# dazchi/gym-uav-collision-avoidance

Hardware: AMD Instinct MI355X
Metric: env-steps/s (higher is better)
Workload: dtype f32+f64

## Files before the change

### gym_uav_collision_avoidance_amd/csrc/uavx_device.hpp

```cpp
#pragma once
#include <hip/hip_runtime.h>
#include <stdint.h>

namespace uavx {

constexpr int kWave = 64;
#ifndef UAVX_BLOCK
#define UAVX_BLOCK 64
#endif
constexpr int kBlock = UAVX_BLOCK;
constexpr int kWavesPerBlock = kBlock / kWave;
constexpr float kPi = 3.14159265358979323846f;
constexpr float kInvPi = 0.318309886183790671538f;
constexpr float kTwoPi = 6.28318530717958647692f;
constexpr float kInvTwoPi = 0.159154943091895335769f;

__device__ __forceinline__ void wave_lds_sync() {
    __builtin_amdgcn_fence(__ATOMIC_RELEASE, "wavefront");
    __builtin_amdgcn_wave_barrier();
    __builtin_amdgcn_fence(__ATOMIC_ACQUIRE, "wavefront");
}

using rsrc_t = __amdgpu_buffer_rsrc_t;
typedef unsigned int u32x4 __attribute__((ext_vector_type(4)));
typedef unsigned int u32x2 __attribute__((ext_vector_type(2)));
constexpr int kAuxSc1 = 16;

__device__ __forceinline__ rsrc_t make_rsrc(const void *base, uint32_t bytes) {
    return __builtin_amdgcn_make_buffer_rsrc(const_cast<void *>(base),  0, (int)bytes, 0x00020000);
}
__device__ __forceinline__ void store16_wt(rsrc_t r, uint32_t byte_off, float4 v) {
    u32x4 d = {__float_as_uint(v.x), __float_as_uint(v.y), __float_as_uint(v.z), __float_as_uint(v.w)};
    __builtin_amdgcn_raw_buffer_store_b128(d, r, (int)byte_off, 0, kAuxSc1);
}
__device__ __forceinline__ void store16_wt(rsrc_t r, uint32_t byte_off, double2 v) {
    const unsigned long long a = __double_as_longlong(v.x), b = __double_as_longlong(v.y);
    u32x4 d = {(unsigned)a, (unsigned)(a >> 32), (unsigned)b, (unsigned)(b >> 32)};
    __builtin_amdgcn_raw_buffer_store_b128(d, r, (int)byte_off, 0, kAuxSc1);
}
__device__ __forceinline__ void store8_wt(rsrc_t r, uint32_t byte_off, float2 v) {
    u32x2 d = {__float_as_uint(v.x), __float_as_uint(v.y)};
    __builtin_amdgcn_raw_buffer_store_b64(d, r, (int)byte_off, 0, kAuxSc1);
}

typedef const __attribute__((address_space(4))) char *karg_ptr;
__device__ __forceinline__ karg_ptr late_kargs() {
    karg_ptr ka = (karg_ptr)__builtin_amdgcn_kernarg_segment_ptr();
    asm volatile("" : "+s"(ka));
    return ka;
}
template <class T>
__device__ __forceinline__ T late_karg(uint32_t byte_off, karg_ptr ka = late_kargs()) {
    return *(const __attribute__((address_space(4))) T *)(ka + byte_off);
}

__device__ __forceinline__ float sqrt_rn(float s) {
    if (__builtin_expect(__any((__float_as_uint(s) - 1u) < 0x0F7FFFFFu), 0)) return sqrtf(s);
    const float r = __builtin_amdgcn_sqrtf(s);
    const float lo = __uint_as_float(__float_as_uint(r) - 1u), hi = __uint_as_float(__float_as_uint(r) + 1u);
    const float e_lo = fmaf(-lo, r, s), e_hi = fmaf(-hi, r, s);
    float out = (e_lo <= 0.f) ? lo : r;
// ... 229 lines not shown
```

### gym_uav_collision_avoidance_amd/csrc/uavx_multi_host.hpp

```cpp

extern "C" {

int uavx_version(void) { return UAVX_VERSION; }

#ifndef UAVX_SRC_HASH
#define UAVX_SRC_HASH ""
#endif
static const char kBuildInfo[] = "UAVX_SRC_HASH=" UAVX_SRC_HASH;
const char *uavx_build_info(void) { return kBuildInfo + 14; }
int uavx_polar_commands(const void *actions, int action_dtype, int64_t n, float scale, double *out, void *stream) {
    if (n < 0 || (n > 0 && (!actions || !out))) return UAVX_ERR_INVALID_ARG;
    if (action_dtype != UAVX_F32 && action_dtype != UAVX_F64) return UAVX_ERR_INVALID_ARG;
    if ((reinterpret_cast<uintptr_t>(actions) & (action_dtype == UAVX_F64 ? 15u : 7u)) || (reinterpret_cast<uintptr_t>(out) & 15u))
        return UAVX_ERR_INVALID_ARG;
    if (n == 0) return UAVX_OK;
    const auto kernel = action_dtype == UAVX_F64 ? &polar_commands_kernel<true> : &polar_commands_kernel<false>;
    return launch_items((uavx_handle *)nullptr, kernel, n, static_cast<hipStream_t>(stream), actions, n, scale, reinterpret_cast<double2 *>(out));
}

const char *uavx_strerror(int status) {
    switch (status) {
        case UAVX_OK: return "ok";
        case UAVX_ERR_INVALID_ARG: return "invalid argument";
        case UAVX_ERR_HIP: return "HIP runtime error";
// ... 29 lines not shown
    h->gw = B > 0 ? 1 : pick_group_waves(N);
    if (const char *gv = getenv("UAVX_GW")) {
        const int w = atoi(gv);
        if (w >= 1 && w <= 4 && B == 0 && !(N == 1 || N == 2 || N == 4 || N == 5 || N == 8)) h->gw = w;
    }
    p.epw = std::min(kWave * h->gw / N, kExtSlots / (N + B));
    p.magic = 65536 / N + 1;
    p.E = num_envs;
    p.env_offset = env_offset;
    h->ext = B > 0;
    {
        const int lps = std::min(kHintJobs, std::max(1, kWave * h->gw / (N + B)));
        h->prefetch_every = std::max(1, 64 * lps / std::max(1, p.epw));
    }
    apply_body_rule(h);
    h->levels.l[0] = make_level(*cfg, nullptr, N, B);

    DeviceGuard guard(device);
    hipError_t e = guard.err;
    if (e != hipSuccess) { delete h; return UAVX_ERR_HIP; }
    const size_t A = (size_t)num_envs * N, E = (size_t)num_envs;
    size_t off = 0;
    const size_t o_pos = off;  off = align_up(off + A * sizeof(float2), 256);
    const size_t o_ovr = off;  off = align_up(off + A * sizeof(float), 256);
    const size_t o_vel = off;  off = align_up(off + A * sizeof(double2), 256);
    const size_t o_goal = off; off = align_up(off + A * sizeof(Goal), 256);
    const size_t o_steps = off; off = align_up(off + E * sizeof(uint4), 256);
    const size_t o_wsteps = off; off = align_up(off + ((E + p.epw - 1) / p.epw) * 4, 256);
    const size_t o_reach = off; off = align_up(off + E * 4, 256);
    const size_t o_coll = off;  off = align_up(off + E * 4, 256);
    const size_t o_nonfin = off; off = align_up(off + E * 4, 256);
    const size_t o_finc = off;  off = align_up(off + E * sizeof(uint4), 256);
    const size_t o_finr = off;  off = align_up(off + E * sizeof(float2), 256);
    const size_t o_bpos = off;  off = align_up(off + E * (size_t)B * sizeof(float2), 256);
    const size_t o_bleg = off;  off = align_up(off + E * (size_t)B * sizeof(float4), 256);
    const size_t o_lcur = off;  off = align_up(off + E, 256);
    const size_t o_lnext = off; off = align_up(off + E, 256);
    const size_t o_levels = off; off = align_up(off + sizeof(LevelTable), 256);
    const size_t o_sagent = off; off = align_up(off + 2 * A * sizeof(float4), 256);
    const size_t o_sbpos = off;  off = align_up(off + 2 * E * (size_t)B * sizeof(float2), 256);
    const size_t o_sbleg = off;  off = align_up(off + 2 * E * (size_t)B * sizeof(float4), 256);
    const size_t o_stag = off;   off = align_up(off + 2 * E * sizeof(uint4), 256);
    const size_t o_hint = off;   off = align_up(off + ((E + p.epw - 1) / p.epw + 1) * kHintJobs * sizeof(uint2), 256);
    static_assert(sizeof(size_t) >= 8, "64-bit host");
    if (o_pos != 0 || o_wsteps >= (size_t(1) << 32)) { delete h; return UAVX_ERR_UNSUPPORTED; }
    h->off_vel = (uint32_t)o_vel; h->off_goal = (uint32_t)o_goal; h->off_rec = (uint32_t)o_steps; h->off_wsteps = (uint32_t)o_wsteps;
    if (p.epw > 255 || p.nslots > 255) { delete h; return UAVX_ERR_UNSUPPORTED; }
    e = hipMalloc(&h->slab, off);
    if (e != hipSuccess) { delete h; return UAVX_ERR_ALLOC; }
    h->slab_bytes = off;
    e = hipMemset(h->slab, 0, off);
    if (e != hipSuccess) { (void)hipFree(h->slab); delete h; return UAVX_ERR_HIP; }
    char *b = static_cast<char *>(h->slab);
    p.pos = reinterpret_cast<float2 *>(b + o_pos);
    p.prev_ovr = reinterpret_cast<float *>(b + o_ovr);
    p.vel = reinterpret_cast<double2 *>(b + o_vel);
    p.goal = reinterpret_cast<Goal *>(b + o_goal);
    p.env_rec = reinterpret_cast<uint4 *>(b + o_steps);
    p.wave_steps = reinterpret_cast<uint32_t *>(b + o_wsteps);
    p.reach = reinterpret_cast<uint32_t *>(b + o_reach);
    p.coll = reinterpret_cast<uint32_t *>(b + o_coll);
    p.nonfin = reinterpret_cast<uint32_t *>(b + o_nonfin);
    p.fin_counts = reinterpret_cast<uint4 *>(b + o_finc);
    p.fin_returns = reinterpret_cast<float2 *>(b + o_finr);
    p.body_pos = reinterpret_cast<float2 *>(b + o_bpos);
    p.body_leg = reinterpret_cast<float4 *>(b + o_bleg);
    p.lvl_cur = reinterpret_cast<uint8_t *>(b + o_lcur);
    p.lvl_next = reinterpret_cast<uint8_t *>(b + o_lnext);
    h->levels_dev = reinterpret_cast<LevelParams *>(b + o_levels);
    p.levels = h->levels_dev;
    p.n_levels = 0; p.level_lo = -1; p.level_hi = -1;
    p.stage_agent = reinterpret_cast<float4 *>(b + o_sagent);
    p.stage_bpos = reinterpret_cast<float2 *>(b + o_sbpos);
    p.stage_bleg = reinterpret_cast<float4 *>(b + o_sbleg);
    p.stage_tag = reinterpret_cast<uint4 *>(b + o_stag);
    h->hints = reinterpret_cast<uint2 *>(b + o_hint);
// ... 129 lines not shown
int uavx_num_agents(const uavx_handle *h) { return h ? h->p.N : -1; }
static int launch_observe(uavx_handle *h, float *obs, hipStream_t st) {
    if (h->wide) return launch_items(h, observe64_kernel, h->p.E, st, h->p, h->w, h->wl, obs);
    return dispatch(h, ObserveLaunch{h, wave_grid(h), st, obs});
}

int uavx_observe(uavx_handle *h, float *obs, void *stream) {
    if (!h) return UAVX_ERR_INVALID_ARG;
    if (!obs || (reinterpret_cast<uintptr_t>(obs) & 15u))
        return fail(h, UAVX_ERR_INVALID_ARG, "uavx_observe: obs is NULL or not 16-byte aligned");
    UAVX_ENTER(h);
    return launch_observe(h, obs, static_cast<hipStream_t>(stream));
}

int uavx_reset(uavx_handle *h, const uint8_t *mask, uint64_t seed, float *obs, void *stream) {
    if (!h) return UAVX_ERR_INVALID_ARG;
    UAVX_ENTER(h);
    if (obs && (reinterpret_cast<uintptr_t>(obs) & 15u))
        return fail(h, UAVX_ERR_INVALID_ARG, "uavx_reset: obs not 16-byte aligned");
    if (h->wide && mask)
        return fail(h, UAVX_ERR_UNSUPPORTED, "uavx_reset: a masked reset would mix float32 and float64 episodes in one handle");
    h->wide = false;
    hipStream_t st = static_cast<hipStream_t>(stream);
    const int rc = dispatch(h, ResetLaunch{h, wave_grid(h), st, mask, seed});
    if (rc != UAVX_OK || !obs) return rc;
    return launch_observe(h, obs, st);
}

static int launch_step64(uavx_handle *h, const void *actions, int action_dtype, int action_mode, int track_returns, int evaluate,
                  float *obs, float *rew, uint8_t *done, hipStream_t st) {
    const bool f64 = action_dtype == UAVX_F64;
    const auto kernel = action_mode == UAVX_ACTION_POLAR_REFERENCE ? (f64 ? &step64_ref_kernel<true> : &step64_ref_kernel<false>)
                                                                   : (f64 ? &step64_kernel<true> : &step64_kernel<false>);
    return launch_items(h, kernel, h->p.E, st, h->p, h->w, h->wl, actions, action_mode, track_returns, evaluate, obs, rew, done);
}

int uavx_step_k(uavx_handle *h, int k, const void *actions, int action_dtype, int evaluate, int tape_out, float *obs,
                float *rew, uint8_t *done, void *stream) {
    if (!h) return UAVX_ERR_INVALID_ARG;
    if (!actions || !obs || !rew || !done) return fail(h, UAVX_ERR_INVALID_ARG, "uavx_step: NULL buffer");
    if (k < 1) return fail(h, UAVX_ERR_INVALID_ARG, "uavx_step_k: k < 1");
    if (action_dtype != UAVX_F32 && action_dtype != UAVX_F64)
        return fail(h, UAVX_ERR_INVALID_ARG, "uavx_step: action_dtype must be UAVX_F32 or UAVX_F64");
    if ((reinterpret_cast<uintptr_t>(obs) & 15u) || (reinterpret_cast<uintptr_t>(actions) & (action_dtype == UAVX_F64 ? 15u : 7u)) ||
        (reinterpret_cast<uintptr_t>(rew) & 3u))
        return fail(h, UAVX_ERR_INVALID_ARG, "uavx_step: obs must be 16-byte aligned, actions 8 (float32) / 16 (float64), rew 4");
    UAVX_ENTER(h);
    if (h->wide) {
        if (k != 1) return fail(h, UAVX_ERR_UNSUPPORTED, "uavx_step_k: k > 1 is not available for float64-position episodes");
        return launch_step64(h, actions, action_dtype, UAVX_ACTION_CARTESIAN, 0, evaluate, obs, rew, done,
                             static_cast<hipStream_t>(stream));
    }
    if (h->ext && k != 1)
        return fail(h, UAVX_ERR_UNSUPPORTED, "uavx_step_k: k > 1 is not available with scripted bodies / a curriculum");
    return dispatch(h, StepLaunch{h, wave_grid(h), static_cast<hipStream_t>(stream), actions, action_dtype, evaluate, k, tape_out, obs, rew, done});
}

int uavx_step(uavx_handle *h, const void *actions, int action_dtype, int evaluate, float *obs, float *rew,
              uint8_t *done, void *stream) {
    return uavx_step_k(h, 1, actions, action_dtype, evaluate, 0, obs, rew, done, stream);
}

int uavx_step_ex(uavx_handle *h, const uavx_step_args *a, void *stream) {
    if (!h || !a) return UAVX_ERR_INVALID_ARG;
    if (!a->actions || !a->obs || !a->rew || !a->done) return fail(h, UAVX_ERR_INVALID_ARG, "uavx_step_ex: NULL buffer");
    if (a->action_dtype != UAVX_F32 && a->action_dtype != UAVX_F64)
        return fail(h, UAVX_ERR_INVALID_ARG, "uavx_step_ex: action_dtype must be UAVX_F32 or UAVX_F64");
    if (a->action_mode != UAVX_ACTION_CARTESIAN && a->action_mode != UAVX_ACTION_POLAR &&
        a->action_mode != UAVX_ACTION_POLAR_REFERENCE)
        return fail(h, UAVX_ERR_INVALID_ARG, "uavx_step_ex: unknown action_mode");
    if (a->reset_policy < UAVX_RESET_NEVER || a->reset_policy > UAVX_RESET_ALL_DONE)
        return fail(h, UAVX_ERR_INVALID_ARG, "uavx_step_ex: unknown reset_policy");
    if (a->flags_mode != UAVX_FLAGS_ARRAYS && a->flags_mode != UAVX_FLAGS_IN_DONE)
        return fail(h, UAVX_ERR_INVALID_ARG, "uavx_step_ex: unknown flags_mode");
    if ((reinterpret_cast<uintptr_t>(a->obs) & 15u) || (reinterpret_cast<uintptr_t>(a->actions) & (a->action_dtype == UAVX_F64 ? 15u : 7u)) ||
        (reinterpret_cast<uintptr_t>(a->rew) & 3u))
        return fail(h, UAVX_ERR_INVALID_ARG, "uavx_step_ex: obs must be 16-byte aligned, actions 8 (float32) / 16 (float64), rew 4");
    UAVX_ENTER(h);
    if (h->wide) {
        if (a->reset_policy != UAVX_RESET_NEVER || a->step_cap != 0)
            return fail(h, UAVX_ERR_UNSUPPORTED, "uavx_step_ex: no auto-reset / step cap for float64-position episodes");
        if (a->reset_mask) UAVX_HIP(h, hipMemsetAsync(a->reset_mask, 0, (size_t)h->p.E, static_cast<hipStream_t>(stream)));
        if (a->ended) UAVX_HIP(h, hipMemsetAsync(a->ended, 0, (size_t)h->p.E, static_cast<hipStream_t>(stream)));
        if (a->truncated) UAVX_HIP(h, hipMemsetAsync(a->truncated, 0, (size_t)h->p.E, static_cast<hipStream_t>(stream)));
        return launch_step64(h, a->actions, a->action_dtype, a->action_mode, a->track_returns, a->evaluate, a->obs, a->rew,
                             a->done, static_cast<hipStream_t>(stream));
    }
    StepExtra x;
    x.action_mode = a->action_mode; x.reset_policy = a->reset_policy; x.track_returns = a->track_returns;
    x.step_cap = a->step_cap; x.seed_lo = (uint32_t)a->seed; x.seed_hi = (uint32_t)(a->seed >> 32);
    x.reset_mask = a->reset_mask;
    x.ended = a->ended; x.truncated = a->truncated;
    x.flags_in_done = (a->flags_mode == UAVX_FLAGS_IN_DONE) ? 1 : 0;
    hipStream_t st = static_cast<hipStream_t>(stream);
    const dim3 grid = wave_grid(h);
    const bool resets = a->reset_policy != UAVX_RESET_NEVER || a->step_cap != 0;
    x.use_stage = (h->prefetch_every > 0 && resets) ? 1 : 0;
    x.pf_blocks = 0; x.pf_groups = grid.x;
    x.stage_first = 0; x.step_first = 0;
    x.hints = h->hints;
    const unsigned step_blocks = grid.x / (unsigned)launch_tiles(h);
// ... 21 lines not shown
}
#endif

int uavx_get_nonfinite(uavx_handle *h, uint32_t *counts, void *stream) {
    if (!h || !counts) return UAVX_ERR_INVALID_ARG;
    UAVX_ENTER(h);
    UAVX_HIP(h, hipMemcpyAsync(counts, h->p.nonfin, (size_t)h->p.E * 4, hipMemcpyDeviceToDevice, static_cast<hipStream_t>(stream)));
    return UAVX_OK;
}

int uavx_get_episode_stats(uavx_handle *h, uint32_t *counts, float *returns, void *stream) {
    if (!h) return UAVX_ERR_INVALID_ARG;
    UAVX_ENTER(h);
    return launch_items(h, episode_stats_kernel, h->p.E, static_cast<hipStream_t>(stream), h->p, counts, returns, 0);
}

int uavx_clear_episode_stats(uavx_handle *h, void *stream) {
    if (!h) return UAVX_ERR_INVALID_ARG;
    UAVX_ENTER(h);
    return launch_items(h, episode_stats_kernel, h->p.E, static_cast<hipStream_t>(stream), h->p, (uint32_t *)nullptr, (float *)nullptr, 1);
}

static int wide_exchange(uavx_handle *h, const uavx_state_view &v, const uavx_state_view_f64 &v64, int set, hipStream_t st) {
    const int rc = launch_items(h, wide_exchange_kernel, agent_slots(h), st, h->p, h->w, v, v64, set);
    if (rc != UAVX_OK || !v.counters) return rc;
    {
        uavx_state_view c;
        std::memset(&c, 0, sizeof c);
        c.counters = v.counters;
        return launch_items(h, set ? set_state_kernel : get_state_kernel, agent_slots(h), st, h->p, c);
    }
}

int uavx_get_state(uavx_handle *h, const uavx_state_view *dst, void *stream) {
    if (!h || !dst) return UAVX_ERR_INVALID_ARG;
    UAVX_ENTER(h);
    if (h->wide) return wide_exchange(h, *dst, uavx_state_view_f64{}, 0, static_cast<hipStream_t>(stream));
    return launch_items(h, get_state_kernel, agent_slots(h), static_cast<hipStream_t>(stream), h->p, *dst);
}

int uavx_set_state(uavx_handle *h, const uavx_state_view *src, void *stream) {
    if (!h || !src) return UAVX_ERR_INVALID_ARG;
    UAVX_ENTER(h);
    if (h->wide) return wide_exchange(h, *src, uavx_state_view_f64{}, 1, static_cast<hipStream_t>(stream));
    return launch_items(h, set_state_kernel, agent_slots(h), static_cast<hipStream_t>(stream), h->p, *src);
}

int uavx_get_position_mode(const uavx_handle *h) { return h ? (h->wide ? UAVX_POS_F64 : UAVX_POS_F32) : UAVX_ERR_INVALID_ARG; }

int uavx_set_position_mode(uavx_handle *h, int mode, void *stream) {
    if (!h) return UAVX_ERR_INVALID_ARG;
    if (mode != UAVX_POS_F32 && mode != UAVX_POS_F64) return fail(h, UAVX_ERR_INVALID_ARG, "uavx_set_position_mode: unknown mode");
    UAVX_ENTER(h);
    if ((mode == UAVX_POS_F64) == h->wide) return UAVX_OK;
    if (mode == UAVX_POS_F64 && h->ext)
        return fail(h, UAVX_ERR_UNSUPPORTED, "uavx_set_position_mode: float64-position episodes are not available with scripted bodies / a curriculum");
    hipStream_t st = static_cast<hipStream_t>(stream);
    if (mode == UAVX_POS_F64) {
        if (!h->wide_slab) {
            const size_t A = (size_t)h->p.E * h->p.N;
            const size_t o_tgt = align_up(A * sizeof(double2), 256), o_init = o_tgt + align_up(A * sizeof(double2), 256);
            const size_t o_prev = o_init + align_up(A * sizeof(double), 256), total = o_prev + align_up(A * sizeof(double), 256);
            if (hipMalloc(&h->wide_slab, total) != hipSuccess) {
                h->wide_slab = nullptr;
                return fail(h, UAVX_ERR_ALLOC, "uavx_set_position_mode: hipMalloc of the float64 arrays failed");
            }
            char *b = static_cast<char *>(h->wide_slab);
            h->w.pos = reinterpret_cast<double2 *>(b);
            h->w.tgt = reinterpret_cast<double2 *>(b + o_tgt);
            h->w.init_d = reinterpret_cast<double *>(b + o_init);
            h->w.prev_d = reinterpret_cast<double *>(b + o_prev);
        }
    }
    const int rc = launch_items(h, mode == UAVX_POS_F64 ? widen_state_kernel : narrow_state_kernel, agent_slots(h), st, h->p, h->w);
    if (rc == UAVX_OK) h->wide = (mode == UAVX_POS_F64);
    return rc;
}

int uavx_set_state_f64(uavx_handle *h, const uavx_state_view_f64 *src, void *stream) {
    if (!h || !src) return UAVX_ERR_INVALID_ARG;
    const int rc = uavx_set_position_mode(h, UAVX_POS_F64, stream);
    if (rc != UAVX_OK) return rc;
    UAVX_ENTER(h);
    uavx_state_view none;
    std::memset(&none, 0, sizeof none);
    return wide_exchange(h, none, *src, 1, static_cast<hipStream_t>(stream));
}

int uavx_get_state_f64(uavx_handle *h, const uavx_state_view_f64 *dst, void *stream) {
    if (!h || !dst) return UAVX_ERR_INVALID_ARG;
    if (!h->wide) return fail(h, UAVX_ERR_UNSUPPORTED, "uavx_get_state_f64: the handle is in float32-position mode");
    UAVX_ENTER(h);
    uavx_state_view none;
    std::memset(&none, 0, sizeof none);
    return wide_exchange(h, none, *dst, 0, static_cast<hipStream_t>(stream));
}
// ... 10 lines not shown
```

### gym_uav_collision_avoidance_amd/csrc/uavx_multi_kernels.hpp

```cpp

#ifndef UAVX_EXB
#define UAVX_EXB 8
#endif
#ifndef UAVX_EX8B
#define UAVX_EX8B 8
#endif
#define UAVX_EX_KERNEL step_ex_kernel
#define UAVX_EX_REF false
#include "uavx_step_ex.hpp"
#undef UAVX_EX_KERNEL
#undef UAVX_EX_REF
#define UAVX_EX_KERNEL step_ex_ref_kernel
#define UAVX_EX_REF true
#include "uavx_step_ex.hpp"
#undef UAVX_EX_KERNEL
#undef UAVX_EX_REF

template <int NT, bool ACT64, int W>
__global__ __launch_bounds__(kWave * W) void step_k_kernel(MultiParams p, const void *__restrict__ actions, int evaluate,
                                                           int K, int tape_out, float *__restrict__ obs_out,
                                                           float *__restrict__ rew_out, uint8_t *__restrict__ done_out) {
    using LDS = LdsT<false, W>;
    __shared__ LDS lds;
    const int N = NT ? NT : p.N;
// ... 10 lines not shown
        float o[10], rew;
        uint32_t dn, re, ce;
        step_agent<NT, false>(p, m, lds, s, ax, ay, evaluate, o, rew, dn, re, ce);
        reach_acc += re;
        coll_acc += ce;
        nonfin_acc += !(fabsf(rew) < INFINITY) ? 1u : 0u;
        if (tape_out || k == K - 1) {
            const size_t off = tape_out ? (size_t)k * A : 0;
            if (m.active) {
                (rew_out + off)[m.a] = rew;
                (done_out + off)[m.a] = (uint8_t)dn;
            }
            store_obs_block<NT>(p, m, lds, o, obs_out + off * UAVX_OBS_DIM);
        } else {
            group_sync<LDS::kW>();
        }
    }
    if (m.active) {
        store_agent(p, m.a, s, flags_in);
        if (reach_acc) atomicAdd(&p.reach[m.e], reach_acc);
        if (coll_acc) atomicAdd(&p.coll[m.e], coll_acc);
        if (nonfin_acc) atomicAdd(&p.nonfin[m.e], nonfin_acc);
        if (m.lane == 0) atomicAdd(&p.wave_steps[m.wave], (uint32_t)K);
    }
}

template <int NT, bool EXT, int W>
__global__ __launch_bounds__(kWave * W) void observe_kernel(MultiParams p, float *__restrict__ obs_out) {
    using LDS = LdsT<EXT, W>;
    __shared__ LDS lds;
    const LaneMap m = lane_map<NT, EXT, W>(p);
    AgentRegs s = {};
    if (m.active) load_agent(p, m.a, s);
    const WorldLims w = world_lims<EXT>(p, s.flags);
    const float tdx = s.tx - s.x, tdy = s.ty - s.y;
    const float dist_t = norm32(tdx, tdy);
    const float theta = atan2_fast((float)s.vy, (float)s.vx);
    const float dth = wrap_pi(atan2_fast(tdy, tdx) - theta);
    if (EXT && p.B > 0) stage_bodies<false>(p, m, lds, s.flags, false, 0u, 0u);
    if (m.active) {
        lds.pos[m.rbase + m.i] = make_float4(s.x, s.y, s.x, s.y);
        lds.theta[m.rbase + m.i] = theta;
    }
    group_sync<LDS::kW>();
    const Neigh nb = scan_neighbours<NT, false>(w.sq_sense, m, lds, s.x, s.y);
    const float speed = __builtin_amdgcn_sqrtf((float)fma(s.vy, s.vy, s.vx * s.vx));
    float o[10];
    assemble_obs(p, w, m, lds, nb, s.x, s.y, speed, theta, dist_t, dth, o);
    if (EXT && (s.flags & kFlagInactive)) {
#pragma unroll
        for (int k = 0; k < UAVX_OBS_DIM; k++) o[k] = 0.f;
    }
    store_obs_block<NT>(p, m, lds, o, obs_out);
}

template <int NT, bool EXT, int W>
__global__ __launch_bounds__(kWave * W) void reset_kernel(MultiParams p, const uint8_t *__restrict__ mask, uint64_t seed) {
    using LDS = LdsT<EXT, W>;
    __shared__ LDS lds;
    const LaneMap m = lane_map<NT, EXT, W>(p);
    const bool go = m.active && (!mask || mask[m.e] != 0);
    if (!group_any<W>(go)) return;
    AgentRegs s = {};
    uint4 rec = make_uint4(0, 0, 0, 0);
    if (go) rec = p.env_rec[m.e];
    const uint32_t episode = rec.y & ~kRecEnded;
    EpisodeFold fold = {};
    uint32_t wc = 0;
    if (go && m.i == 0) {
        fold = fold_load(p, m.e);
        wc = p.wave_steps[m.wave];
    }
    reset_envs_wave<NT, EXT>(p, m, lds, go, episode, (uint32_t)seed, (uint32_t)(seed >> 32), s, p.body_pos, p.body_leg, p.lvl_cur);
    if (go) {
        p.pos[m.a] = make_float2(s.x, s.y);
        p.vel[m.a] = make_double2(0.0, 0.0);
        p.goal[m.a] = Goal{s.tx, s.ty, s.init_d, s.flags};
        if (m.i == 0) {
            fold_store(p, m.e, wc - rec.x, make_float2(__uint_as_float(rec.z), __uint_as_float(rec.w)), fold);
            p.env_rec[m.e] = make_uint4(wc, episode + 1u, 0u, 0u);
        }
    }
}

__global__ __launch_bounds__(64) void upload_levels_kernel(LevelParams *dst, LevelTable t) {
    if (threadIdx.x < UAVX_MAX_LEVELS) dst[threadIdx.x] = t.l[threadIdx.x];
}
__global__ __launch_bounds__(kBlock) void env_levels_kernel(MultiParams p, const uint8_t *set_next, uint8_t *get_cur) {
    const int64_t e = (int64_t)blockIdx.x * kBlock + threadIdx.x;
    if (e >= p.E) return;
    if (set_next) p.lvl_next[e] = set_next[e];
    if (get_cur) get_cur[e] = p.lvl_cur[e];
}
__global__ __launch_bounds__(kBlock) void bodies_kernel(MultiParams p, const float *set, float *get) {
    const int64_t i = (int64_t)blockIdx.x * kBlock + threadIdx.x;
    if (i >= p.E * p.B) return;
    if (set) {
        const float *r = set + i * UAVX_BODY_DIM;
        p.body_pos[i] = make_float2(r[0], r[1]);
        p.body_leg[i] = make_float4(r[2], r[3], r[4], r[5]);
    }
    if (get) {
        const float2 q = p.body_pos[i];
        const float4 leg = p.body_leg[i];
        float *r = get + i * UAVX_BODY_DIM;
// ... 106 lines not shown
```

### gym_uav_collision_avoidance_amd/csrc/uavx_multi_launch.hpp

```cpp

namespace {

template <class L>
int dispatch(const uavx_handle *h, const L &l) {
    if (h->ext) {
        switch (h->gw) {
            case 2: return l.template run<0, true, 2>();
            case 3: return l.template run<0, true, 3>();
            case 4: return l.template run<0, true, 4>();
            default: return l.template run<0, true, 1>();
        }
    }
    switch (h->p.N) {
        case 1: return l.template run<1, false, 1>();
        case 2: return l.template run<2, false, 1>();
        case 4: return l.template run<4, false, 1>();
        case 5: return l.template run<5, false, 1>();
        case 8: return l.template run<8, false, 1>();
        default: break;
    }
    switch (h->gw) {
        case 2: return l.template run<0, false, 2>();
        case 3: return l.template run<0, false, 3>();
        case 4: return l.template run<0, false, 4>();
// ... 60 lines not shown
    template <int NT, bool EXT, int W> int run() const {
        return launch(h, reset_kernel<NT, EXT, W>, grid, dim3(kWave * W), st, h->p, mask, seed);
    }
};

int pick_group_waves(int N) {
    if (N == 1 || N == 2 || N == 4 || N == 5 || N == 8) return 1;
    switch (N) {
        case 3: case 6: case 7: case 11: case 12: case 24: case 48: return 3;
        case 9: case 10: case 15: case 20: case 40: return 2;
        case 13: case 14: case 16: case 28: case 32: case 64: return 1;
        default: break;
    }
    const double u1 = (double)((kWave / N) * N) / kWave;
    double best = u1;
    int w = 1;
    for (int c = 2; c <= 4; c++) {
        const double u = (double)((kWave * c / N) * N) / (kWave * c);
        if (u > best + 1e-9) { best = u; w = c; }
    }
    return best > 1.10 * u1 ? w : 1;
}

dim3 wave_grid(const uavx_handle *h) {
    return dim3((unsigned)((h->p.E + h->p.epw - 1) / h->p.epw));
}
inline int64_t agent_slots(const uavx_handle *h) { return h->p.E * h->p.N; }

}
```

### gym_uav_collision_avoidance_amd/csrc/uavx_multi_scan.hpp

```cpp

struct LaneMap {
    int lane;
    int i, base;
    int rbase, nslots;
    int nlearn;
    int g;
    bool active;
    uint32_t e, a;
    uint32_t a0;
    uint32_t wave;
    int obs0;
    int cnt;
};

template <int NT, bool EXT = false, int W = 1>
__device__ __forceinline__ LaneMap lane_map_from(uint32_t E, int n_agents, int envs_per_group, int magic, int nslots, uint32_t wave,
                                                 uint32_t lane = threadIdx.x, uint32_t tile = 0u) {
    LaneMap m;
    const int N = NT ? NT : n_agents;
    const int epw = NT ? (kWave / (NT ? NT : 1)) : envs_per_group;
    m.lane = lane;
    int g;
    if (NT) {
        g = m.lane / (NT ? NT : 1);
// ... 18 lines not shown
    m.cnt = (int)envs_here * N;
    return m;
}
template <int NT, bool EXT = false, int W = 1>
__device__ __forceinline__ LaneMap lane_map(const MultiParams &p, uint32_t wave = blockIdx.x) {
    return lane_map_from<NT, EXT, W>((uint32_t)p.E, p.N, p.epw, p.magic, p.nslots, wave);
}

struct AgentRegs {
    float x, y, prev_d;
    uint32_t flags;
    float tx, ty, init_d;
    double vx, vy;
};

template <bool EXT, int W = 1>
struct LdsT {
    static constexpr int kW = W;
    static constexpr int kRows = (EXT && kExtSlots > kWave * W) ? kExtSlots : kWave * W;
    float4 pos[kRows];
    float theta[kRows];
    float obs[kWave * W * UAVX_OBS_DIM];
};
template <>
struct LdsT<true, 1> {
    static constexpr int kW = 1;
    static constexpr int kRows = kExtSlots;
    union {
        struct {
            float4 pos[kRows];
            float theta[kRows];
        };
        float obs[kWave * UAVX_OBS_DIM];
    };
};
template <int W>
__device__ __forceinline__ void group_sync() {
    if (W == 1) wave_lds_sync();
    else __syncthreads();
}
template <int W>
__device__ __forceinline__ bool group_any(bool v) {
    if (W == 1) return __ballot(v) != 0ull;
    return __syncthreads_or(v ? 1 : 0) != 0;
}
using Lds = LdsT<false>;
// ... 9 lines not shown
template <bool EXT>
__device__ __forceinline__ float sense_limit(const MultiParams &p, uint32_t flags) {
    if (EXT && p.n_levels > 0) return p.levels[(flags & kLevelMask) >> kLevelShift].sq_sense;
    return p.sq_sense;
}
template <bool EXT>
__device__ __forceinline__ WorldLims world_lims(const MultiParams &p, uint32_t flags) {
    WorldLims w;
    if (EXT && p.n_levels > 0) {
        const float4 *t = reinterpret_cast<const float4 *>(&p.levels[(flags & kLevelMask) >> kLevelShift]);
        const float4 a = t[0], b = t[1];
        w.lo_x = a.x; w.lo_y = a.y; w.hi_x = a.z; w.hi_y = a.w;
        w.sq_sense = b.x; w.sq_two_r = b.y; w.inv_sense = b.z; w.inv_diag = b.w;
    } else {
        w.lo_x = p.lo_x; w.lo_y = p.lo_y; w.hi_x = p.hi_x; w.hi_y = p.hi_y;
        w.sq_sense = p.sq_sense; w.sq_two_r = p.sq_two_r; w.inv_sense = p.inv_sense; w.inv_diag = p.inv_diag;
    }
    return w;
}

__device__ __forceinline__ float natural_prev_d(uint32_t flags, float x, float y, float tx, float ty) {
    const float d = norm32(tx - x, ty - y);
    return ((flags & UAVX_FLAG_DONE) && !(flags & kFlagJustDone)) ? 0.f : d;
}

__device__ __forceinline__ void load_agent(const MultiParams &p, uint32_t a, AgentRegs &s) {
    const float2 d = p.pos[a];
    const double2 v = p.vel[a];
    const Goal g = p.goal[a];
    s.x = d.x; s.y = d.y;
    s.vx = v.x; s.vy = v.y;
    s.tx = g.tx; s.ty = g.ty; s.init_d = g.init_d; s.flags = g.flags;
    s.prev_d = natural_prev_d(s.flags, s.x, s.y, s.tx, s.ty);
    if (s.flags & kFlagPrevOvr) s.prev_d = p.prev_ovr[a];
}
__device__ __forceinline__ void store_agent(const MultiParams &p, float2 *pos, double2 *vel, Goal *goal, uint32_t a,
                                            const AgentRegs &s, uint32_t flags_in) {
    store16_wt(make_rsrc(vel, (uint32_t)p.E * (uint32_t)p.N * 16u), a * 16u, make_double2(s.vx, s.vy));
    pos[a] = make_float2(s.x, s.y);
    if (s.flags != flags_in) goal[a].flags = s.flags;
}
__device__ __forceinline__ void store_agent(const MultiParams &p, uint32_t a, const AgentRegs &s, uint32_t flags_in) {
    store_agent(p, p.pos, p.vel, p.goal, a, s, flags_in);
}

struct Neigh {
// ... 247 lines not shown
```

### gym_uav_collision_avoidance_amd/csrc/uavx_multi_step.hpp

```cpp

template <class LDS>
__device__ __forceinline__ void assemble_obs(const MultiParams &p, const WorldLims &w, const LaneMap &m, const LDS &lds,
                                             const Neigh &nb, float nx, float ny, float speed, float theta, float dist_t,
                                             float dth, float o[10]) {
    o[0] = speed * p.inv_vmax_norm;
    o[1] = theta * kInvPi;
    o[2] = dist_t * w.inv_diag;
    o[3] = dth * kInvPi;
    const bool has1 = nb.j1 >= 0, has2 = nb.j2 >= 0;
    const int i1 = m.rbase + (has1 ? nb.j1 : 0), i2 = m.rbase + (has2 ? nb.j2 : 0);
    const float4 q1 = lds.pos[i1], q2 = lds.pos[i2];
    const float t1 = lds.theta[i1], t2 = lds.theta[i2];
    const float b1 = wrap_unit(atan2_fast(q1.w - ny, q1.z - nx) - theta);
    const float b2 = wrap_unit(atan2_fast(q2.w - ny, q2.z - nx) - theta);
    const float h1 = wrap_unit(t1 - theta);
    const float h2 = wrap_unit(t2 - theta);
    o[4] = has1 ? nb.d1 * w.inv_sense : 1.f;
    o[5] = has1 ? b1 : 1.f;
    o[6] = has1 ? h1 : 0.f;
    o[7] = has2 ? nb.d2 * w.inv_sense : 1.f;
    o[8] = has2 ? b2 : 1.f;
    o[9] = has2 ? h2 : 0.f;
}

// ... 166 lines not shown
    }
}

template <bool ACT64>
__device__ __forceinline__ void load_action(const void *__restrict__ actions, uint32_t a, double &ax, double &ay) {
    if (ACT64) {
        const double2 v = reinterpret_cast<const double2 *>(actions)[a];
        ax = v.x; ay = v.y;
    } else {
        const float2 v = reinterpret_cast<const float2 *>(actions)[a];
        ax = (double)v.x; ay = (double)v.y;
    }
}

#ifndef UAVX_STEPB
#define UAVX_STEPB 8
#endif
template <int NT, bool ACT64, bool EXT, int W, int T = 1>
__global__ __launch_bounds__(kWave * W * T, (EXT && W == 1) ? UAVX_STEPB : 1) void step_kernel(
    const void *__restrict__ actions, char *slab, uint32_t off_vel, uint32_t off_goal, uint32_t off_rec, uint32_t off_wsteps,
    uint32_t num_envs, uint32_t n_agents, uint32_t envs_per_group, uint32_t magic, uint32_t nslots, MultiParams p, int evaluate,
    float *__restrict__ obs_out, float *__restrict__ rew_out, uint8_t *__restrict__ done_out) {
    static_assert(T == 1 || W == 1, "tiles are one-wavefront workgroups side by side");
    using LDS = std::conditional_t<(T > 1), LdsTiles<T>, LdsT<EXT, W>>;
    static_assert(T == 1 || !EXT, "tiles: the plain variants only");
    __shared__ LDS lds;
    const uint32_t tile = T > 1 ? (uint32_t)__builtin_amdgcn_readfirstlane((int)(threadIdx.x / kWave)) : 0u;
    constexpr bool BUF = NT == 4 && !EXT && T == 1;
    float2 *const pos_b = reinterpret_cast<float2 *>(slab);
    double2 *const vel_b = reinterpret_cast<double2 *>(slab + off_vel);
    Goal *const goal_b = reinterpret_cast<Goal *>(slab + off_goal);
    const uint32_t nslot = num_envs * n_agents;
    const rsrc_t r_act = make_rsrc(actions, nslot * (ACT64 ? 16u : 8u));
    const rsrc_t r_pos = make_rsrc(slab, nslot * 8u), r_vel = make_rsrc(slab + off_vel, nslot * 16u);
    const rsrc_t r_goal = make_rsrc(slab + off_goal, nslot * 16u);
    const uint32_t wave_id = blockIdx.x * T + tile;
    const LaneMap m = lane_map_from<NT, EXT, W>(num_envs, (int)n_agents, (int)envs_per_group, (int)magic, (int)nslots, wave_id,
                                                T > 1 ? threadIdx.x % kWave : threadIdx.x, tile);
    AgentRegs s = {};
    double ax = 0.0, ay = 0.0;
    uint4 rec = make_uint4(0, 0, 0, 0);
    uint32_t wave_count = 0;
    {
        const uint32_t el = m.active ? m.e : 0u, al = m.active ? m.a : 0u;
        if (EXT) {
            rec = reinterpret_cast<const uint4 *>(slab + off_rec)[el];
            wave_count = reinterpret_cast<const uint32_t *>(slab + off_wsteps)[wave_id];
        }
        if (!BUF) {
            load_action<ACT64>(actions, al, ax, ay);
            const float2 d = pos_b[al];
            const double2 v = vel_b[al];
            const Goal g = goal_b[al];
            __builtin_amdgcn_sched_barrier(0);
            s.x = d.x; s.y = d.y; s.vx = v.x; s.vy = v.y;
            s.tx = g.tx; s.ty = g.ty; s.init_d = g.init_d; s.flags = g.flags;
        } else {
            if (ACT64) {
                const u32x4 c = __builtin_amdgcn_raw_buffer_load_b128(r_act, al * 16u, 0, 0);
                ax = __hiloint2double(c.y, c.x); ay = __hiloint2double(c.w, c.z);
            } else {
                const u32x2 c = __builtin_amdgcn_raw_buffer_load_b64(r_act, al * 8u, 0, 0);
                ax = (double)__uint_as_float(c.x); ay = (double)__uint_as_float(c.y);
            }
            const u32x2 d = __builtin_amdgcn_raw_buffer_load_b64(r_pos, al * 8u, 0, 0);
            const u32x4 v = __builtin_amdgcn_raw_buffer_load_b128(r_vel, al * 16u, 0, 0);
            const u32x4 g = __builtin_amdgcn_raw_buffer_load_b128(r_goal, al * 16u, 0, 0);
            __builtin_amdgcn_sched_barrier(0);
            s.x = __uint_as_float(d.x); s.y = __uint_as_float(d.y);
            s.vx = __hiloint2double(v.y, v.x); s.vy = __hiloint2double(v.w, v.z);
            s.tx = __uint_as_float(g.x); s.ty = __uint_as_float(g.y); s.init_d = __uint_as_float(g.z); s.flags = g.w;
        }
        s.prev_d = natural_prev_d(s.flags, s.x, s.y, s.tx, s.ty);
        if (m.active && (s.flags & kFlagPrevOvr)) s.prev_d = p.prev_ovr[m.a];
    }
    const uint32_t flags_in = s.flags;
    float o[10], rew;
    uint32_t dn, re, ce;
    step_agent<NT, EXT, LDS, false, BUF>(p, m, lds, s, ax, ay, evaluate, o, rew, dn, re, ce, false, wave_count - rec.x,
                                    ((rec.y & ~kRecEnded) - 1u) & ~kRecEnded);
    if (m.active) {
        if (!BUF) {
            if (!(EXT && (flags_in & kFlagInactive))) store_agent(p, pos_b, vel_b, goal_b, m.a, s, flags_in);
            rew_out[m.a] = rew;
            done_out[m.a] = (uint8_t)dn;
        } else {
            store16_wt(r_vel, m.a * 16u, make_double2(s.vx, s.vy));
            const u32x2 d = {__float_as_uint(s.x), __float_as_uint(s.y)};
            __builtin_amdgcn_raw_buffer_store_b64(d, r_pos, m.a * 8u, 0, 0);
            if (s.flags != flags_in) __builtin_amdgcn_raw_buffer_store_b32(s.flags, r_goal, m.a * 16u + 12u, 0, 0);
            __builtin_amdgcn_raw_buffer_store_b32(__float_as_uint(rew), make_rsrc(rew_out, nslot * 4u), m.a * 4u, 0, 0);
            __builtin_amdgcn_raw_buffer_store_b8((uint8_t)dn, make_rsrc(done_out, nslot), m.a, 0, 0);
        }
        if (re) atomicAdd(&p.reach[m.e], 1u);
        if (ce) atomicAdd(&p.coll[m.e], 1u);
        if (!(fabsf(rew) < INFINITY)) atomicAdd(&p.nonfin[m.e], 1u);
        if (m.lane == 0) {
            uint32_t *const ws = reinterpret_cast<uint32_t *>(slab + off_wsteps);
            if (EXT) ws[m.wave] = wave_count + 1u;
            else atomicAdd(&ws[m.wave], 1u);
        }
    }
    store_obs_block<NT>(p, m, lds, o, obs_out);
}
```

### gym_uav_collision_avoidance_amd/csrc/uavx_step_ex.hpp

```cpp
template <int NT, bool ACT64, bool EXT, int W, int T = 1>
__global__ __launch_bounds__(kWave * W * T, (W != 1) ? 1 : (EXT ? UAVX_EXB : (NT == 8 ? UAVX_EX8B : 1))) void UAVX_EX_KERNEL(const void *__restrict__ actions, char *slab, uint32_t off_vel, uint32_t off_goal,
                                                            uint32_t off_rec, uint32_t off_wsteps, uint32_t num_envs, uint32_t stage_first,
                                                            uint32_t pf_blocks, uint32_t step_first, uint32_t shape_packed, uint32_t magic,
                                                            MultiParams p, StepExtra x, int evaluate,
                                                            float *__restrict__ obs_out, float *__restrict__ rew_out_arg,
                                                            uint8_t *__restrict__ done_out_arg) {
    static_assert(kExLead == 2 * sizeof(void *) + 10 * sizeof(uint32_t), "leading scalar arguments of step_ex_kernel");
    static_assert(T == 1 || W == 1, "tiles are one-wavefront workgroups side by side");
    using LDS = std::conditional_t<(T > 1), LdsTiles<T>, LdsT<EXT, W>>;
    static_assert(T == 1 || !EXT, "tiles: the plain variants only");
    __shared__ LDS lds;
    const uint32_t tile = T > 1 ? (uint32_t)__builtin_amdgcn_readfirstlane((int)(threadIdx.x / kWave)) : 0u;
    const int N = NT ? NT : (int)(shape_packed & 0xFFu);
    float2 *const pos_b = reinterpret_cast<float2 *>(slab);
    double2 *const vel_b = reinterpret_cast<double2 *>(slab + off_vel);
    Goal *const goal_b = reinterpret_cast<Goal *>(slab + off_goal);
    uint4 *const rec_b = reinterpret_cast<uint4 *>(slab + off_rec);
    uint32_t *const wsteps_b = reinterpret_cast<uint32_t *>(slab + off_wsteps);
    constexpr bool kTight = (EXT || NT == 8) && W == 1;
    constexpr int kLate = kTight ? UAVX_LATE_EX : 0;
    constexpr bool kLateR = (kLate & 8) != 0;
    {
        const uint32_t sb = blockIdx.x - stage_first;
        if (sb < pf_blocks) {
// ... 173 lines not shown
    uint8_t *done_out = done_out_arg;
    if constexpr (kLateR && UAVX_LATE) {
        LATE_BASE(true, kt);
        pos_p = LATE_AT(true, kt, p, pos); vel_p = LATE_AT(true, kt, p, vel); goal_p = LATE_AT(true, kt, p, goal);
        rec_p = LATE_AT(true, kt, p, env_rec); wsteps_p = LATE_AT(true, kt, p, wave_steps);
        rew_out = late_karg<float *>(kIoRew, kt); done_out = late_karg<uint8_t *>(kIoDone, kt);
    }
    if (m.active) {
        if (!(EXT && (s.flags & kFlagInactive))) store_agent(p, pos_p, vel_p, goal_p, m.a, s, flags_in);
        else if (do_reset) { pos_p[m.a] = make_float2(s.x, s.y); vel_p[m.a] = make_double2(0.0, 0.0); }
        rew_out[m.a] = rew;
        const uint32_t steps_next = do_reset ? 0u : steps_v + 1u;
        const bool terminal = (x.reset_policy == UAVX_RESET_AGENT0_DONE && dn != 0) ||
                              (x.reset_policy == UAVX_RESET_ALL_DONE && all_done);
        const bool capped = x.step_cap != 0 && steps_next >= x.step_cap;
        const bool ended = (terminal || capped) && !do_reset;
        uint32_t dbyte = dn;
        if (x.flags_in_done && m.i == 0) dbyte |= (do_reset ? 2u : 0u) | (ended ? 4u : 0u) | ((ended && !terminal) ? 8u : 0u);
        done_out[m.a] = (uint8_t)dbyte;
        if (re) atomicAdd(&LATE(kLate & 1, p, reach)[m.e], 1u);
        if (ce) atomicAdd(&LATE(kLate & 1, p, coll)[m.e], 1u);
        if (!(fabsf(rew) < INFINITY)) atomicAdd(&LATE(kLate & 1, p, nonfin)[m.e], 1u);
        if (m.lane == 0) wsteps_p[m.wave] = wave_count + 1u;
        if (m.i == 0) {
            const uint4 rec = (EXT || NT == 8) ? rec_p[m.e] : rec0;
            float2 run = do_reset ? make_float2(0.f, 0.f) : make_float2(__uint_as_float(rec.z), __uint_as_float(rec.w));
            if (!x.flags_in_done) {
                uint8_t *const rm = LATE_X(kLateR, x, reset_mask), *const en = LATE_X(kLateR, x, ended), *const tr = LATE_X(kLateR, x, truncated);
                if (rm) rm[m.e] = do_reset ? 1 : 0;
                if (en) en[m.e] = ended ? 1 : 0;
                if (tr) tr[m.e] = (ended && !terminal) ? 1 : 0;
            }
            uint4 out = rec;
            if (do_reset) {
                fold_store<(kLate & 4) != 0>(p, m.e, wave_count - rec.x, make_float2(__uint_as_float(rec.z), __uint_as_float(rec.w)),
                                             fold_load<(kLate & 4) != 0>(p, m.e));
                out.x = wave_count + 1u;
                out.y = episode + 1u;
            }
            out.y = (out.y & ~kRecEnded) | (ended ? kRecEnded : 0u);
            if (x.track_returns) {
                float score = 0.f;
                for (int j = 0; j < N; j++) score += lds.theta[m.rbase + j];
                run.x += do_reset ? 0.f : rew;
                run.y += score;
            }
// ... 10 lines not shown
```

Baseline: 11.46 billion.

## Carry prev distance across N=4 steps with generation invalidation and coalesce rew/done stores

For the N=4 non-extended step kernel, each agent's previous goal distance is now stored in a persistent buffer and reloaded on the next step instead of being recomputed. A per-wave generation counter, bumped by resets, state sets, mode changes and other kernels, marks the carried value stale so it falls back to the natural value. Rewards and done bytes are staged in LDS and written as full 16-byte rows when a wavefront is full and the outputs are aligned. The state buffer descriptors are merged into one resource with scalar offsets. This adds bookkeeping launches on several host paths and extra global traffic for the carry value and generation check.

```diff
diff --git a/gym_uav_collision_avoidance_amd/csrc/uavx_device.hpp b/gym_uav_collision_avoidance_amd/csrc/uavx_device.hpp
--- a/gym_uav_collision_avoidance_amd/csrc/uavx_device.hpp
+++ b/gym_uav_collision_avoidance_amd/csrc/uavx_device.hpp
@@ -37,6 +37,11 @@
     const unsigned long long a = __double_as_longlong(v.x), b = __double_as_longlong(v.y);
     u32x4 d = {(unsigned)a, (unsigned)(a >> 32), (unsigned)b, (unsigned)(b >> 32)};
     __builtin_amdgcn_raw_buffer_store_b128(d, r, (int)byte_off, 0, kAuxSc1);
+}
+__device__ __forceinline__ void store16_wt_at(rsrc_t r, uint32_t scalar_off, uint32_t byte_off, double2 v) {
+    const unsigned long long a = __double_as_longlong(v.x), b = __double_as_longlong(v.y);
+    u32x4 d = {(unsigned)a, (unsigned)(a >> 32), (unsigned)b, (unsigned)(b >> 32)};
+    __builtin_amdgcn_raw_buffer_store_b128(d, r, (int)byte_off, (int)scalar_off, kAuxSc1);
 }
 __device__ __forceinline__ void store8_wt(rsrc_t r, uint32_t byte_off, float2 v) {
     u32x2 d = {__float_as_uint(v.x), __float_as_uint(v.y)};
diff --git a/gym_uav_collision_avoidance_amd/csrc/uavx_multi_host.hpp b/gym_uav_collision_avoidance_amd/csrc/uavx_multi_host.hpp
--- a/gym_uav_collision_avoidance_amd/csrc/uavx_multi_host.hpp
+++ b/gym_uav_collision_avoidance_amd/csrc/uavx_multi_host.hpp
@@ -75,7 +75,7 @@
     const size_t A = (size_t)num_envs * N, E = (size_t)num_envs;
     size_t off = 0;
     const size_t o_pos = off;  off = align_up(off + A * sizeof(float2), 256);
-    const size_t o_ovr = off;  off = align_up(off + A * sizeof(float), 256);
+    const size_t o_ovr = off;  off = align_up(align_up(off + A * sizeof(float), 256) + (kPrevGenWave + (E + p.epw - 1) / p.epw) * 4, 256);
     const size_t o_vel = off;  off = align_up(off + A * sizeof(double2), 256);
     const size_t o_goal = off; off = align_up(off + A * sizeof(Goal), 256);
     const size_t o_steps = off; off = align_up(off + E * sizeof(uint4), 256);
@@ -105,6 +105,8 @@
     e = hipMemset(h->slab, 0, off);
     if (e != hipSuccess) { (void)hipFree(h->slab); delete h; return UAVX_ERR_HIP; }
     char *b = static_cast<char *>(h->slab);
+    e = hipMemset(b + o_ovr + align_up(A * sizeof(float), 256), 1, 1);
+    if (e != hipSuccess) { (void)hipFree(h->slab); delete h; return UAVX_ERR_HIP; }
     p.pos = reinterpret_cast<float2 *>(b + o_pos);
     p.prev_ovr = reinterpret_cast<float *>(b + o_ovr);
     p.vel = reinterpret_cast<double2 *>(b + o_vel);
@@ -280,6 +282,7 @@
         return fail(h, UAVX_ERR_UNSUPPORTED, "uavx_reset: a masked reset would mix float32 and float64 episodes in one handle");
     h->wide = false;
     hipStream_t st = static_cast<hipStream_t>(stream);
+    if (!keeps_prev_carry(h)) { const int rc = drop_prev_carry(h, st); if (rc != UAVX_OK) return rc; }
     const int rc = dispatch(h, ResetLaunch{h, wave_grid(h), st, mask, seed});
     if (rc != UAVX_OK || !obs) return rc;
     return launch_observe(h, obs, st);
@@ -304,6 +307,7 @@
         (reinterpret_cast<uintptr_t>(rew) & 3u))
         return fail(h, UAVX_ERR_INVALID_ARG, "uavx_step: obs must be 16-byte aligned, actions 8 (float32) / 16 (float64), rew 4");
     UAVX_ENTER(h);
+    if (!keeps_prev_carry(h)) { const int rc = drop_prev_carry(h, static_cast<hipStream_t>(stream)); if (rc != UAVX_OK) return rc; }
     if (h->wide) {
         if (k != 1) return fail(h, UAVX_ERR_UNSUPPORTED, "uavx_step_k: k > 1 is not available for float64-position episodes");
         return launch_step64(h, actions, action_dtype, UAVX_ACTION_CARTESIAN, 0, evaluate, obs, rew, done,
@@ -335,6 +339,7 @@
         (reinterpret_cast<uintptr_t>(a->rew) & 3u))
         return fail(h, UAVX_ERR_INVALID_ARG, "uavx_step_ex: obs must be 16-byte aligned, actions 8 (float32) / 16 (float64), rew 4");
     UAVX_ENTER(h);
+    if (!keeps_prev_carry(h)) { const int rc = drop_prev_carry(h, static_cast<hipStream_t>(stream)); if (rc != UAVX_OK) return rc; }
     if (h->wide) {
         if (a->reset_policy != UAVX_RESET_NEVER || a->step_cap != 0)
             return fail(h, UAVX_ERR_UNSUPPORTED, "uavx_step_ex: no auto-reset / step cap for float64-position episodes");
@@ -402,6 +407,7 @@
 }
 
 static int wide_exchange(uavx_handle *h, const uavx_state_view &v, const uavx_state_view_f64 &v64, int set, hipStream_t st) {
+    if (set) { const int rc = drop_prev_carry(h, st); if (rc != UAVX_OK) return rc; }
     const int rc = launch_items(h, wide_exchange_kernel, agent_slots(h), st, h->p, h->w, v, v64, set);
     if (rc != UAVX_OK || !v.counters) return rc;
     {
@@ -423,6 +429,7 @@
     if (!h || !src) return UAVX_ERR_INVALID_ARG;
     UAVX_ENTER(h);
     if (h->wide) return wide_exchange(h, *src, uavx_state_view_f64{}, 1, static_cast<hipStream_t>(stream));
+    { const int rc = drop_prev_carry(h, static_cast<hipStream_t>(stream)); if (rc != UAVX_OK) return rc; }
     return launch_items(h, set_state_kernel, agent_slots(h), static_cast<hipStream_t>(stream), h->p, *src);
 }
 
@@ -452,6 +459,7 @@
             h->w.prev_d = reinterpret_cast<double *>(b + o_prev);
         }
     }
+    { const int rc = drop_prev_carry(h, st); if (rc != UAVX_OK) return rc; }
     const int rc = launch_items(h, mode == UAVX_POS_F64 ? widen_state_kernel : narrow_state_kernel, agent_slots(h), st, h->p, h->w);
     if (rc == UAVX_OK) h->wide = (mode == UAVX_POS_F64);
     return rc;
diff --git a/gym_uav_collision_avoidance_amd/csrc/uavx_multi_kernels.hpp b/gym_uav_collision_avoidance_amd/csrc/uavx_multi_kernels.hpp
--- a/gym_uav_collision_avoidance_amd/csrc/uavx_multi_kernels.hpp
+++ b/gym_uav_collision_avoidance_amd/csrc/uavx_multi_kernels.hpp
@@ -56,6 +56,7 @@
         if (coll_acc) atomicAdd(&p.coll[m.e], coll_acc);
         if (nonfin_acc) atomicAdd(&p.nonfin[m.e], nonfin_acc);
         if (m.lane == 0) atomicAdd(&p.wave_steps[m.wave], (uint32_t)K);
+        if (NT == 4 && m.a == 0u) drop_prev_gen(p);
     }
 }
 
@@ -94,6 +95,7 @@
     __shared__ LDS lds;
     const LaneMap m = lane_map<NT, EXT, W>(p);
     const bool go = m.active && (!mask || mask[m.e] != 0);
+    if (NT == 4 && !EXT && blockIdx.x == 0 && threadIdx.x == 0) drop_prev_gen(p);
     if (!group_any<W>(go)) return;
     AgentRegs s = {};
     uint4 rec = make_uint4(0, 0, 0, 0);
@@ -115,6 +117,10 @@
             p.env_rec[m.e] = make_uint4(wc, episode + 1u, 0u, 0u);
         }
     }
+}
+
+__global__ __launch_bounds__(64) void prev_gen_kernel(MultiParams p) {
+    if (threadIdx.x == 0) drop_prev_gen(p);
 }
 
 __global__ __launch_bounds__(64) void upload_levels_kernel(LevelParams *dst, LevelTable t) {
diff --git a/gym_uav_collision_avoidance_amd/csrc/uavx_multi_launch.hpp b/gym_uav_collision_avoidance_amd/csrc/uavx_multi_launch.hpp
--- a/gym_uav_collision_avoidance_amd/csrc/uavx_multi_launch.hpp
+++ b/gym_uav_collision_avoidance_amd/csrc/uavx_multi_launch.hpp
@@ -106,6 +106,12 @@
     return best > 1.10 * u1 ? w : 1;
 }
 
+int drop_prev_carry(uavx_handle *h, hipStream_t st) {
+    if (h->p.N != 4) return UAVX_OK;
+    return launch(h, prev_gen_kernel, dim3(1), dim3(64), st, h->p);
+}
+inline bool keeps_prev_carry(const uavx_handle *h) { return h->p.N == 4 && !h->ext && !h->wide; }
+
 dim3 wave_grid(const uavx_handle *h) {
     return dim3((unsigned)((h->p.E + h->p.epw - 1) / h->p.epw));
 }
diff --git a/gym_uav_collision_avoidance_amd/csrc/uavx_multi_scan.hpp b/gym_uav_collision_avoidance_amd/csrc/uavx_multi_scan.hpp
--- a/gym_uav_collision_avoidance_amd/csrc/uavx_multi_scan.hpp
+++ b/gym_uav_collision_avoidance_amd/csrc/uavx_multi_scan.hpp
@@ -64,6 +64,14 @@
     float theta[kRows];
     float obs[kWave * W * UAVX_OBS_DIM];
 };
+struct LdsStep4 {
+    static constexpr int kW = 1;
+    float4 pos[kWave];
+    float theta[kWave];
+    uint4 tail[kWave / 4 + kWave / 16];
+    float obs[kWave * UAVX_OBS_DIM];
+};
+static_assert(offsetof(LdsStep4, obs) == offsetof(LdsStep4, tail) + 320 && sizeof(LdsStep4::obs) >= (kWave - 20) * 16, "tail rows");
 template <>
 struct LdsT<true, 1> {
     static constexpr int kW = 1;
@@ -119,6 +127,14 @@
 __device__ __forceinline__ float natural_prev_d(uint32_t flags, float x, float y, float tx, float ty) {
     const float d = norm32(tx - x, ty - y);
     return ((flags & UAVX_FLAG_DONE) && !(flags & kFlagJustDone)) ? 0.f : d;
+}
+
+constexpr uint32_t kPrevGenWave = 64;
+__device__ __forceinline__ uint32_t *prev_gen(float *prev_ovr, uint32_t nslot) {
+    return reinterpret_cast<uint32_t *>(prev_ovr) + ((nslot + 63u) & ~63u);
+}
+__device__ __forceinline__ void drop_prev_gen(const MultiParams &p) {
+    atomicAdd(prev_gen(p.prev_ovr, (uint32_t)p.E * (uint32_t)p.N), 1u);
 }
 
 __device__ __forceinline__ void load_agent(const MultiParams &p, uint32_t a, AgentRegs &s) {
diff --git a/gym_uav_collision_avoidance_amd/csrc/uavx_multi_step.hpp b/gym_uav_collision_avoidance_amd/csrc/uavx_multi_step.hpp
--- a/gym_uav_collision_avoidance_amd/csrc/uavx_multi_step.hpp
+++ b/gym_uav_collision_avoidance_amd/csrc/uavx_multi_step.hpp
@@ -212,19 +212,22 @@
     uint32_t num_envs, uint32_t n_agents, uint32_t envs_per_group, uint32_t magic, uint32_t nslots, MultiParams p, int evaluate,
     float *__restrict__ obs_out, float *__restrict__ rew_out, uint8_t *__restrict__ done_out) {
     static_assert(T == 1 || W == 1, "tiles are one-wavefront workgroups side by side");
-    using LDS = std::conditional_t<(T > 1), LdsTiles<T>, LdsT<EXT, W>>;
+    constexpr bool BUF = NT == 4 && !EXT && T == 1;
+    constexpr bool CARRY = BUF, ROWS = BUF;
+    using LDS = std::conditional_t<(T > 1), LdsTiles<T>, std::conditional_t<ROWS, LdsStep4, LdsT<EXT, W>>>;
     static_assert(T == 1 || !EXT, "tiles: the plain variants only");
     __shared__ LDS lds;
     const uint32_t tile = T > 1 ? (uint32_t)__builtin_amdgcn_readfirstlane((int)(threadIdx.x / kWave)) : 0u;
-    constexpr bool BUF = NT == 4 && !EXT && T == 1;
     float2 *const pos_b = reinterpret_cast<float2 *>(slab);
     double2 *const vel_b = reinterpret_cast<double2 *>(slab + off_vel);
     Goal *const goal_b = reinterpret_cast<Goal *>(slab + off_goal);
     const uint32_t nslot = num_envs * n_agents;
     const rsrc_t r_act = make_rsrc(actions, nslot * (ACT64 ? 16u : 8u));
-    const rsrc_t r_pos = make_rsrc(slab, nslot * 8u), r_vel = make_rsrc(slab + off_vel, nslot * 16u);
-    const rsrc_t r_goal = make_rsrc(slab + off_goal, nslot * 16u);
+    const rsrc_t r_st = make_rsrc(slab, off_goal + nslot * 16u);
     const uint32_t wave_id = blockIdx.x * T + tile;
+    const uint32_t off_prev = (nslot * 8u + 255u) & ~255u, off_gen = off_prev + ((nslot * 4u + 255u) & ~255u);
+    uint32_t prev_in = 0;
+    bool stale = false;
     const LaneMap m = lane_map_from<NT, EXT, W>(num_envs, (int)n_agents, (int)envs_per_group, (int)magic, (int)nslots, wave_id,
                                                 T > 1 ? threadIdx.x % kWave : threadIdx.x, tile);
     AgentRegs s = {};
@@ -253,34 +256,67 @@
                 const u32x2 c = __builtin_amdgcn_raw_buffer_load_b64(r_act, al * 8u, 0, 0);
                 ax = (double)__uint_as_float(c.x); ay = (double)__uint_as_float(c.y);
             }
-            const u32x2 d = __builtin_amdgcn_raw_buffer_load_b64(r_pos, al * 8u, 0, 0);
-            const u32x4 v = __builtin_amdgcn_raw_buffer_load_b128(r_vel, al * 16u, 0, 0);
-            const u32x4 g = __builtin_amdgcn_raw_buffer_load_b128(r_goal, al * 16u, 0, 0);
+            const u32x2 d = __builtin_amdgcn_raw_buffer_load_b64(r_st, al * 8u, 0, 0);
+            const u32x4 v = __builtin_amdgcn_raw_buffer_load_b128(r_st, al * 16u, off_vel, 0);
+            const u32x4 g = __builtin_amdgcn_raw_buffer_load_b128(r_st, al * 16u, off_goal, 0);
+            if (CARRY) {
+                prev_in = __builtin_amdgcn_raw_buffer_load_b32(r_st, al * 4u, off_prev, 0);
+                const uint32_t *const gw = reinterpret_cast<const uint32_t *>(slab + off_gen);
+                stale = gw[0] != gw[kPrevGenWave + wave_id];
+            }
             __builtin_amdgcn_sched_barrier(0);
             s.x = __uint_as_float(d.x); s.y = __uint_as_float(d.y);
             s.vx = __hiloint2double(v.y, v.x); s.vy = __hiloint2double(v.w, v.z);
             s.tx = __uint_as_float(g.x); s.ty = __uint_as_float(g.y); s.init_d = __uint_as_float(g.z); s.flags = g.w;
         }
-        s.prev_d = natural_prev_d(s.flags, s.x, s.y, s.tx, s.ty);
-        if (m.active && (s.flags & kFlagPrevOvr)) s.prev_d = p.prev_ovr[m.a];
+        if (CARRY) {
+            s.prev_d = __uint_as_float(prev_in);
+            if (stale) {
+                const float nat = norm32(s.tx - s.x, s.ty - s.y);
+                if (!(s.flags & kFlagPrevOvr)) s.prev_d = nat;
+                if (m.lane == 0)
+                    __builtin_amdgcn_raw_buffer_store_b32(__builtin_amdgcn_raw_buffer_load_b32(r_st, 0, off_gen, 0), r_st,
+                                                          (kPrevGenWave + wave_id) * 4u, off_gen, 0);
+            }
+        } else {
+            s.prev_d = natural_prev_d(s.flags, s.x, s.y, s.tx, s.ty);
+            if (m.active && (s.flags & kFlagPrevOvr)) s.prev_d = p.prev_ovr[m.a];
+        }
     }
     const uint32_t flags_in = s.flags;
     float o[10], rew;
     uint32_t dn, re, ce;
     step_agent<NT, EXT, LDS, false, BUF>(p, m, lds, s, ax, ay, evaluate, o, rew, dn, re, ce, false, wave_count - rec.x,
                                     ((rec.y & ~kRecEnded) - 1u) & ~kRecEnded);
+    const auto full_rows = [&]() {
+        uint32_t off16 = ((uint32_t)reinterpret_cast<uintptr_t>(rew_out) | (uint32_t)reinterpret_cast<uintptr_t>(done_out)) & 15u;
+        asm volatile("" : "+s"(off16));
+        return ROWS && m.cnt == kWave && off16 == 0u;
+    };
+    const bool rows = full_rows();
     if (m.active) {
         if (!BUF) {
             if (!(EXT && (flags_in & kFlagInactive))) store_agent(p, pos_b, vel_b, goal_b, m.a, s, flags_in);
             rew_out[m.a] = rew;
             done_out[m.a] = (uint8_t)dn;
         } else {
-            store16_wt(r_vel, m.a * 16u, make_double2(s.vx, s.vy));
+            store16_wt_at(r_st, off_vel, m.a * 16u, make_double2(s.vx, s.vy));
             const u32x2 d = {__float_as_uint(s.x), __float_as_uint(s.y)};
-            __builtin_amdgcn_raw_buffer_store_b64(d, r_pos, m.a * 8u, 0, 0);
-            if (s.flags != flags_in) __builtin_amdgcn_raw_buffer_store_b32(s.flags, r_goal, m.a * 16u + 12u, 0, 0);
-            __builtin_amdgcn_raw_buffer_store_b32(__float_as_uint(rew), make_rsrc(rew_out, nslot * 4u), m.a * 4u, 0, 0);
-            __builtin_amdgcn_raw_buffer_store_b8((uint8_t)dn, make_rsrc(done_out, nslot), m.a, 0, 0);
+            __builtin_amdgcn_raw_buffer_store_b64(d, r_st, m.a * 8u, 0, 0);
+            if (s.flags != flags_in) __builtin_amdgcn_raw_buffer_store_b32(s.flags, r_st, m.a * 16u + 12u, off_goal, 0);
+            if (CARRY) {
+                __builtin_amdgcn_raw_buffer_store_b32(__float_as_uint(s.prev_d), r_st, m.a * 4u, off_prev, 0);
+            }
+            if constexpr (ROWS) {
+                if (rows) {
+                    reinterpret_cast<float *>(lds.tail)[m.lane] = rew;
+                    reinterpret_cast<uint8_t *>(lds.tail)[kWave * 4 + m.lane] = (uint8_t)dn;
+                }
+            }
+            if (!rows) {
+                __builtin_amdgcn_raw_buffer_store_b32(__float_as_uint(rew), make_rsrc(rew_out, nslot * 4u), m.a * 4u, 0, 0);
+                __builtin_amdgcn_raw_buffer_store_b8((uint8_t)dn, make_rsrc(done_out, nslot), m.a, 0, 0);
+            }
         }
         if (re) atomicAdd(&p.reach[m.e], 1u);
         if (ce) atomicAdd(&p.coll[m.e], 1u);
@@ -292,4 +328,16 @@
         }
     }
     store_obs_block<NT>(p, m, lds, o, obs_out);
-}
+    if constexpr (ROWS) {
+        if (full_rows()) {
+            constexpr int kRewRows = kWave / 4, kRows = kWave / 4 + kWave / 16;
+            int ln = m.lane;
+            asm volatile("" : "+v"(ln));
+            const uint4 v = *reinterpret_cast<const uint4 *>(reinterpret_cast<const char *>(lds.tail) + ln * 16);
+            const u32x4 d = {v.x, v.y, v.z, v.w};
+            if (ln < kRewRows) __builtin_amdgcn_raw_buffer_store_b128(d, make_rsrc(rew_out + m.a0, kWave * 4u), ln * 16, 0, 0);
+            if ((unsigned)(ln - kRewRows) < (unsigned)(kRows - kRewRows))
+                __builtin_amdgcn_raw_buffer_store_b128(d, make_rsrc(done_out + m.a0 - kWave * 4, kWave * 5u), ln * 16, 0, 0);
+        }
+    }
+}
diff --git a/gym_uav_collision_avoidance_amd/csrc/uavx_step_ex.hpp b/gym_uav_collision_avoidance_amd/csrc/uavx_step_ex.hpp
--- a/gym_uav_collision_avoidance_amd/csrc/uavx_step_ex.hpp
+++ b/gym_uav_collision_avoidance_amd/csrc/uavx_step_ex.hpp
@@ -219,6 +219,7 @@
         if (ce) atomicAdd(&LATE(kLate & 1, p, coll)[m.e], 1u);
         if (!(fabsf(rew) < INFINITY)) atomicAdd(&LATE(kLate & 1, p, nonfin)[m.e], 1u);
         if (m.lane == 0) wsteps_p[m.wave] = wave_count + 1u;
+        if (NT == 4 && !EXT && m.a == 0u) drop_prev_gen(p);
         if (m.i == 0) {
             const uint4 rec = (EXT || NT == 8) ? rec_p[m.e] : rec0;
             float2 run = do_reset ? make_float2(0.f, 0.f) : make_float2(__uint_as_float(rec.z), __uint_as_float(rec.w));
```

After: 11.43 billion. No clear change (-0.3%).
